# ArroyoSystems/arroyo

Measured on NVIDIA H100. Metric: rows/sec sliding-window SUM (1M keys), higher is better.
Workload: dtype int64

## Files before the change

arroyo_b200/csrc/ingest_two_pass.cuh:

```cuda
#pragma once

struct alignas(16) Rec {
  long long key;
  long long val;
};

constexpr int TP_NP = 2;
#ifndef AB_P1_THREADS
#define AB_P1_THREADS 512
#endif
#ifndef AB_P1_RPT
#define AB_P1_RPT 8
#endif
constexpr int P1_THREADS = AB_P1_THREADS;
constexpr int P1_RPT = AB_P1_RPT;
constexpr int P1_TILE = P1_THREADS * P1_RPT;
constexpr int P1_NWARP = P1_THREADS / 32;
constexpr int P1_NR = 1024;
constexpr int P1_BLOCKS_PER_SM = P1_TILE <= 4096 ? 2 : 1;
constexpr int P2_NW = 16;
constexpr int P2_NST = 3;
constexpr int P2_CH = 64;
constexpr int P2_BLOCKS_PER_SM = 2;
constexpr uint32_t NO_REGION = 0xFFFFu;

struct TwoPassParams {
  unsigned long long fast_q[TP_NP];
  unsigned long long* fast_ptr[TP_NP];
  uint32_t fast_slot[TP_NP];
  Rec* part;
  unsigned int* cursor;
  unsigned int* cursor_next;
  uint32_t cap;
  uint32_t slices;
  uint32_t tail_first;
  uint32_t tail_slices;
};

constexpr size_t P1_SMEM = (size_t)P1_TILE * 16 + (size_t)P1_NR * 12;
constexpr size_t P2_SMEM = (size_t)4096 * 11 + (size_t)BD_CAPB * 12 + (size_t)P2_NW * P2_NST * P2_CH * 16 +
                           (size_t)(P2_NW * P2_NST + 1) * 8;

template <int NV>
__device__ __noinline__ void direct_rec(const IngestParams& p, unsigned long long* pane, uint32_t slot, uint64_t q,
                                        long long key, long long val) {
  if (NV > 0 && p.guard_vals && big_one(val)) {
    atomicAdd(&p.counters->big_vals, 1ull);
// ... 132 lines not shown
#pragma unroll
    for (int o = 1; o < 32; o <<= 1) {
      const uint32_t y = __shfl_up_sync(0xffffffffu, incl, o);
      if (lane >= o) incl += y;
    }
    if (lane == 31) s_wsum[w] = incl;
    __syncthreads();
    uint32_t wbase = 0, n_on = 0;
#pragma unroll
    for (int ww = 0; ww < P1_NWARP; ++ww) {
      const uint32_t x = s_wsum[ww];
      if (ww < w) wbase += x;
      n_on += x;
    }
    const uint32_t ex0 = wbase + incl - tsum;
    uint32_t g[BPT];
    {
      uint32_t ex = ex0;
      const uint32_t rbase = (uint32_t)max(psel, 0) * NB;
#pragma unroll
      for (int x = 0; x < BPT; ++x) {
        const uint32_t b = BPT * tid + x;
        toff[b] = ex;
        g[x] = 0;
        if (c[x]) g[x] = atomicAdd(tp.cursor + rbase + b, c[x]);
        ex += c[x];
      }
    }
    __syncthreads();

// ... 12 lines not shown
        gdelta[BPT * tid + x] = g[x] - ex;
        ex += c[x];
      }
    }
    __syncthreads();
    if (n_on) {
      Rec* out = tp.part + (size_t)max(psel, 0) * NB * tp.cap;
      for (uint32_t i = tid; i < n_on; i += P1_THREADS) {
        const Rec rec = reorder[i];
        const uint32_t r = bd_bucket(bd_hash(rec.key), NB);
        const uint32_t dst = gdelta[r] + i;
        if (dst < tp.cap) {
          out[(size_t)r * tp.cap + dst] = rec;
        } else {
          atomicAdd(&p.counters->part_overflow, 1ull);
          direct_rec<NV>(p, fpane, fslot, tq, rec.key, rec.val);
        }
      }
    }
  }

  unsigned long long wl = late;
#pragma unroll
  for (int o = 16; o > 0; o >>= 1) {
    wl += __shfl_xor_sync(0xffffffffu, wl, o);
    maxq = max(maxq, __shfl_xor_sync(0xffffffffu, maxq, o));
  }
  if (lane == 0) {
    if (wl) atomicAdd(&s_late, wl);
    if (maxq) atomicMax(&s_maxq, (unsigned long long)maxq);
// ... 94 lines not shown
  uint32_t sl = (g + P2_HG) & (P2_HS - 1);
#pragma unroll 1
  for (int probe = 0; full && probe < P2_HS; ++probe) {
    const unsigned long long e = hk[sl];
    if (e == (unsigned long long)key && htag[sl] != 0) return hidx[sl];
    if (e == (unsigned long long)EMPTY_KEY) break;
    sl = (sl + 1) & (P2_HS - 1);
  }
  const uint32_t id = bd_insert(p.dict, b, key, bd_slot0(key));
  if (id >= ID_OVERFLOW) return ID_OVERFLOW;
  const uint32_t idx = id - bd_id(b, 0);
  p2_insert(hk, htag, hidx, key, idx);
  return idx;
}

__device__ __noinline__ void agg_defer(const IngestParams& p, long long key, long long ts, long long val, int why) {
  if (why == 0) atomicAdd(&p.counters->big_vals, 1ull);
  else atomicAdd(&p.counters->dict_full, 1u);
  defer_row(p, key, ts, val, 0, 0, 0);
}

constexpr unsigned P2_FLUSH_ITERS = 31;

template <int NV>
__global__ void __launch_bounds__(P2_NW * 32, P2_BLOCKS_PER_SM) agg_kernel(const __grid_constant__ IngestParams p,
                                                                           const __grid_constant__ TwoPassParams tp) {
  extern __shared__ __align__(128) unsigned char smem_raw[];
  unsigned long long* hk = reinterpret_cast<unsigned long long*>(smem_raw);
  unsigned char* htag = reinterpret_cast<unsigned char*>(hk + P2_HS);
  unsigned short* hidx = reinterpret_cast<unsigned short*>(htag + P2_HS);
  uint32_t* scw = reinterpret_cast<uint32_t*>(hidx + P2_HS);
  uint32_t* slo = scw + BD_CAPB;
  uint32_t* shi = slo + BD_CAPB;
  Rec* ring = reinterpret_cast<Rec*>(shi + BD_CAPB);
  unsigned long long* bars = reinterpret_cast<unsigned long long*>(ring + (size_t)P2_NW * P2_NST * P2_CH);
  __shared__ unsigned long long s_rows;
  const int tid = threadIdx.x, lane = tid & 31, w = tid >> 5;
  const uint32_t NB = p.dict.n_buckets;
  Rec* myring = ring + (size_t)w * P2_NST * P2_CH;
  const uint32_t bar0 = smem_u32(bars + (size_t)w * P2_NST);
  const uint32_t a_hk = smem_u32(hk), a_tag = smem_u32(htag), a_idx = smem_u32(hidx), a_cw = smem_u32(scw),
                 a_lo = smem_u32(slo), a_hi = smem_u32(shi), a_ring = smem_u32(myring);
  if (lane == 0)
    for (int s = 0; s < P2_NST; ++s) mbar_init(bar0 + 8 * s, 1);
  asm volatile("fence.mbarrier_init.release.cluster;" ::: "memory");
  for (int i = tid; i < 3 * BD_CAPB; i += P2_NW * 32) scw[i] = 0;
  if (tid == 0) s_rows = 0;
  __syncthreads();
  uint32_t phase = 0;
  const bool guard = NV > 0 && p.guard_vals != 0;

  const uint32_t head_work = tp.tail_first * tp.slices;
  const uint32_t n_work = head_work + (NB - tp.tail_first) * tp.tail_slices;
  for (uint32_t work = blockIdx.x; work < n_work; work += gridDim.x) {
    const bool tail = work >= head_work;
    const uint32_t n_slices = tail ? tp.tail_slices : tp.slices;
    const uint32_t b = tail ? tp.tail_first + (work - head_work) / n_slices : work / n_slices;
    const uint32_t slice = tail ? (work - head_work) % n_slices : work % n_slices;
    unsigned n_reg[TP_NP];
    unsigned n_any = 0;
#pragma unroll
    for (int f = 0; f < TP_NP; ++f) {
      n_reg[f] = tp.fast_ptr[f] ? min(tp.cursor[f * NB + b], tp.cap) : 0u;
      n_any |= n_reg[f];
      if (tid == 0) tp.cursor_next[f * NB + b] = 0;
    }
    if (n_any == 0) continue;

    const Rec* rows = nullptr;
    unsigned n = 0, my_chunks = 0;
    auto select = [&](int f) {
      const unsigned chunks_all = (n_reg[f] + P2_CH - 1) / P2_CH;
      const unsigned c_lo = (unsigned)((unsigned long long)chunks_all * slice / n_slices);
      const unsigned c_hi = (unsigned)((unsigned long long)chunks_all * (slice + 1) / n_slices);
      const unsigned r_lo = c_lo * P2_CH, r_hi = min(c_hi * P2_CH, n_reg[f]);
      rows = tp.part + (size_t)(f * NB + b) * tp.cap + r_lo;
      n = r_hi > r_lo ? r_hi - r_lo : 0u;
      const unsigned n_chunks = (n + P2_CH - 1) / P2_CH;
      my_chunks = n_chunks > (unsigned)w ? (n_chunks - w + P2_NW - 1) / P2_NW : 0;
    };
// ... 21 lines not shown
      }
    }
    __syncthreads();

#pragma unroll 1
    for (int f = 0; f < TP_NP; ++f) {
      if (f > 0) {
        select(f);
        for (unsigned ci = 0; ci < (unsigned)P2_NST && ci < my_chunks; ++ci) issue(ci, (int)ci);
      }
      if (n == 0) continue;
      unsigned long long* pane = tp.fast_ptr[f];
      const long long pane_ts = (long long)(tp.fast_q[f] * (uint64_t)p.slide);
      unsigned long long* prow = pane + bd_id(b, 0);
      unsigned long long* psum = pane + p.id_cap + bd_id(b, 0);
      unsigned int flushed = 0;
      auto flush = [&]() {
        for (unsigned i = tid; i < (unsigned)BD_CAPB; i += P2_NW * 32) {
          const uint32_t cw = scw[i];
          if (cw) {
            const uint32_t c = cw & 0xFFFFu;
            const uint32_t dh = (uint32_t)((int32_t)(cw - c) >> 16);
            const unsigned long long sum = ((unsigned long long)(shi[i] + dh) << 32) + (unsigned long long)slo[i];
            scw[i] = 0;
            slo[i] = 0;
            shi[i] = 0;
            flushed += c;
            if (n_slices == 1) {
              prow[i] += c;
              if (NV > 0) psum[i] += sum;
            } else {
              red_add_u64(prow + i, c);
              if (NV > 0) red_add_u64(psum + i, sum);
            }
          }
        }
      };
      const unsigned iters = ((n + P2_CH - 1) / P2_CH + P2_NW - 1) / P2_NW;
#pragma unroll 1
      for (unsigned ci = 0; ci < iters; ++ci) {
        if (ci && ci % P2_FLUSH_ITERS == 0) {
          __syncthreads();
          flush();
          __syncthreads();
        }
        if (ci >= my_chunks) continue;
        const int s = (int)(ci % P2_NST);
        mbar_wait(bar0 + 8 * s, (phase >> s) & 1u);
        phase ^= 1u << s;
// ... 15 lines not shown
            while (m) {
              const uint32_t bit = (uint32_t)__ffs(m) - 1u;
              m &= m - 1;
              const uint32_t j = (bit >> 3) + (bit & 4u);
              if ((uint32_t)((tg >> (8 * j)) & 0xFFull) != (tag4 & 0xFFu)) continue;
              const uint32_t sl = g + j;
              if (lds64(a_hk + sl * 8) == (unsigned long long)key) {
                idx = lds16(a_idx + sl * 2);
                break;
              }
            }
            if (idx == ID_UNSET) idx = agg_slow_lookup(p, hk, htag, hidx, b, key, g);
            const uint32_t vl = rr.z, vh = rr.w;
            const bool narrow = NV == 0 || (uint32_t)((int32_t)vl >> 31) == vh;
            if (idx >= (uint32_t)BD_CAPB) {
              agg_defer(p, key, pane_ts, (long long)(((unsigned long long)vh << 32) | vl), 1);
            } else if (NV > 0 && guard && !narrow) {
              agg_defer(p, key, pane_ts, (long long)(((unsigned long long)vh << 32) | vl), 0);
            } else if (NV == 0) {
              reds_add(a_cw + idx * 4, 1u);
            } else {
              const uint32_t old = atoms_add(a_lo + idx * 4, vl);
              uint32_t d = (old + vl) < vl ? 1u : 0u;
              if (narrow) d -= vl >> 31;
              else reds_add(a_hi + idx * 4, vh);
              reds_add(a_cw + idx * 4, 1u + (d << 16));
            }
          }
        }
        __syncwarp();
        if (ci + P2_NST < my_chunks) issue(ci + P2_NST, s);
      }
      __syncthreads();
      flush();
      flushed = __reduce_add_sync(0xffffffffu, flushed);
      if (lane == 0 && flushed) atomicAdd(&s_rows, (unsigned long long)flushed);
      __syncthreads();
      if (tid == 0) {
        if (s_rows) atomicAdd(p.slot_rows + tp.fast_slot[f], s_rows);
        s_rows = 0;
      }
    }
    __syncthreads();
  }
}
```

arroyo_b200/csrc/window_agg.cu:

```cuda
#include <algorithm>
#include <climits>
#include <deque>
#include <map>
#include <memory>
#include <set>

#include "agg_plan.h"
#include "bdict.cuh"
#include "op.h"
#include "planner.h"

namespace ab {
namespace {

constexpr int MAX_SEGS = 512;
constexpr int MAX_RING = 4096;
constexpr int RING_INLINE = 64;
constexpr int MAX_MERGE = 4096;
constexpr long long FREE_BIN = LLONG_MIN;

constexpr int THREADS = 256;
constexpr int PAIRS = 2;
constexpr int TILE = THREADS * PAIRS * 2;

// ... 682 lines not shown
  int slot = -1;
  bool in_tier = false;
  uint64_t rows = 0;
  bool exported = false;
  bool delta_exported = false;
};

struct LaunchRec {
  cudaEvent_t done = nullptr;
  cudaEvent_t t0 = nullptr, t1 = nullptr;
  Counters* h_counters = nullptr;
  unsigned long long* h_slot_rows = nullptr;
  uint64_t rows = 0;
  bool in_flight = false;
  int chunk = -1;
};

constexpr size_t RELEASE_GROUP = 16;
struct PendingRelease {
  cudaEvent_t ev;
  std::vector<ArrowArray> arrs;
};

class WindowAggOp final : public OpBase {
 public:
  explicit WindowAggOp(const ArroyoB200OpConfig& c);
  ~WindowAggOp() override;

  void on_start(ArrowArray* state, ArrowSchema* schemas, int64_t n, int64_t watermark, int64_t table_min) override;
  void process_batch(uint32_t, uint32_t, ArrowArray* batch, const ArrowSchema* schema) override;
// ... 28 lines not shown
  static constexpr size_t BOOK_SLOT_OFF = (sizeof(Counters) + 15) / 16 * 16;
  Counters* d_counters() const { return reinterpret_cast<Counters*>(book_.p); }
  unsigned long long* d_slot_rows() const { return reinterpret_cast<unsigned long long*>((char*)book_.p + BOOK_SLOT_OFF); }
  std::vector<unsigned long long> slot_rows_seen_;
  uint32_t n_keys_host_ = 1;
  uint32_t total_keys_host_ = 0;
  uint32_t dict_full_seen_ = 0;
  DevBuf part_, part_cursor_;
  uint32_t part_cap_ = 0;
  int part_flip_ = 0;
  bool two_pass_attr_set_ = false;
  bool two_pass_enabled_ = true;
  uint64_t part_overflow_seen_ = 0;
  mutable int two_pass_pause_ = 0;
  bool two_pass_eligible(uint64_t rows) const;
  void launch_two_pass(IngestParams& p, uint64_t rows, long long tiles_direct);
  BDict dict_view() const;
  cudaStream_t out_stream_ = nullptr;
  cudaEvent_t emit_done_ = nullptr, out_done_ = nullptr;
  bool async_out_ = false, out_inflight_ = false;
  void wait_outputs();
  static constexpr size_t COPY_GROUP = 48;
  std::vector<void*> copy_dst_, copy_src_;
  std::vector<size_t> copy_size_;
  bool batch_copy_ok_ = true;
  void queue_copy(void* dst, const void* src, size_t bytes);
  void flush_copies();
  std::vector<ArrowArray> open_release_;
  std::vector<cudaEvent_t> ev_pool_;
  void seal_release();

// ... 72 lines not shown
  void preallocate();
  void grow_ids();
  void apply_l2_policy();
  void promote_avg();
  void relayout_blocks(int old_n_acc, const std::vector<std::pair<int, int>>& f64_from);
  unsigned long long* acquire_block();
  void release_block(unsigned long long* blk);
  void init_block(unsigned long long* blk, uint64_t n_ids);
  void ensure_pane(int64_t bin);
  void drop_pane(int64_t bin);
  void upload_ring();
  void add_segment(const long long* key, const long long* ts, const long long* const* vals, int64_t n);
  void launch_pending();
  void launch_segments(const std::vector<Segment>& segs, int chunk);
  void absorb(int li);
  void sync_all();
  void drain_deferred();
  void poll_releases(bool wait);
  void rotate_chunk();
  void touch(int64_t bin);
  OutSet* out_set(size_t i, uint64_t cap);
  int64_t run_emit(const std::vector<const unsigned long long*>& blocks, int n_add, bool use_running, bool partial,
                   int64_t wstart, int64_t wend, int64_t ts, OutSet* os);
  void emit_window(int64_t a, int64_t b, size_t out_index, BatchesPriv* out_host,
                   std::vector<ArroyoB200DeviceBatch>* out_dev);
  void export_window(OutSet* os, int64_t n, BatchesPriv* out_host);
  void export_partial(OutSet* os, int64_t n, BatchesPriv* out);
  void collect_emit_times();
  void lookahead();
};

// ... 36 lines not shown

  book_.alloc(BOOK_SLOT_OFF + MAX_RING * sizeof(unsigned long long));
  AB_CUDA(cudaMemsetAsync(book_.p, 0, book_.bytes, stream_));
  slot_rows_seen_.assign(MAX_RING, 0);
  Counters init{};
  init.max_q = 0;
  init.n_keys = 0;
  AB_CUDA(cudaMemcpyAsync(book_.p, &init, sizeof init, cudaMemcpyHostToDevice, stream_));
  last_counters_ = init;

  uint64_t want = c.expected_keys ? c.expected_keys : (1ull << 16);
  alloc_dictionary(plan_.keyed ? bd_buckets_for(want) : 1);
  {
    const char* e = getenv("ARROYO_B200_NO_TWO_PASS");
    two_pass_enabled_ = !(e && atoi(e) != 0) && !(c.flags & ARROYO_B200_FLAG_NO_TWO_PASS);
  }

  h_pane_bins_.assign(MAX_RING, FREE_BIN);
  h_pane_ptrs_.assign(MAX_RING, nullptr);
  d_pane_bins_.alloc(MAX_RING * sizeof(long long));
  d_pane_ptrs_.alloc(MAX_RING * sizeof(void*));
  if (sliding_) {
    uint64_t need = (uint64_t)(width_ / slide_) + 8;
    while (ring_ < need && ring_ < MAX_RING) ring_ <<= 1;
  }

  const int n_used = 2 + plan_.n_vals;
  for (int i = 0; i < NCHUNK; ++i) {
    AB_CUDA(cudaEventCreateWithFlags(&chunk_free_[i], cudaEventDisableTiming));
    if (i == 0) {
// ... 36 lines not shown
    auto* blk = pane_storage_.back().as<unsigned long long>();
    init_block(blk, id_cap_);
    free_panes_.emplace_back(blk, 0);
  }
  for (int c = 0; c < 2 + plan_.n_vals; ++c) defer_[0][c].alloc(defer_cap_ * 8);
  out_set(0, id_cap_);
  out_set(1, id_cap_);
}

WindowAggOp::~WindowAggOp() {
  cudaSetDevice(device_);
  if (counts_done_) cudaEventDestroy(counts_done_);
  if (copy_stream_) cudaStreamSynchronize(copy_stream_);
  if (out_stream_) cudaStreamSynchronize(out_stream_);
  cudaStreamSynchronize(stream_);
  for (auto& r : releases_) {
    for (auto& a : r.arrs)
      if (a.release) a.release(&a);
    cudaEventDestroy(r.ev);
  }
  for (auto& a : zero_copy_inputs_)
    if (a.release) a.release(&a);
  for (auto& a : open_release_)
    if (a.release) a.release(&a);
  for (auto e : ev_pool_) cudaEventDestroy(e);
  for (int i = 0; i < NCHUNK; ++i)
    if (chunk_free_[i]) cudaEventDestroy(chunk_free_[i]);
  if (copy_stream_) {
    cudaStreamSynchronize(copy_stream_);
    cudaStreamDestroy(copy_stream_);
// ... 98 lines not shown

__global__ void permute_block_kernel(const unsigned long long* __restrict__ old_blk, unsigned long long* __restrict__ new_blk,
                                     const uint32_t* __restrict__ map, uint32_t old_ids, uint64_t old_cap, uint64_t new_cap,
                                     int n_acc) {
  uint32_t i = blockIdx.x * blockDim.x + threadIdx.x;
  const uint32_t stride = gridDim.x * blockDim.x;
  for (; i < old_ids; i += stride) {
    const uint32_t m = map[i];
    if (m == ID_UNSET || m >= ID_OVERFLOW) continue;
    for (int a = 0; a < n_acc; ++a) new_blk[(uint64_t)a * new_cap + m] = old_blk[(uint64_t)a * old_cap + i];
  }
}

void WindowAggOp::grow_ids() {
  AB_REQUIRE(plan_.keyed, ARROYO_B200_RUNTIME, "grow_ids on an unkeyed aggregate");
  const uint64_t old_cap = id_cap_;
  const uint32_t old_ids = n_keys_host_;
  BDict old_d = dict_view();
  DevBuf old_slots = std::move(slots_), old_nkeys = std::move(bucket_nkeys_), old_keys = std::move(id_keys_);
  old_d.slots = old_slots.as<BSlot>();
  old_d.nkeys = old_nkeys.as<unsigned int>();
  old_d.id_keys = old_keys.as<long long>();
  const unsigned int zero = 0;
  AB_CUDA(cudaMemcpyAsync((char*)book_.p + offsetof(Counters, n_keys), &zero, sizeof zero, cudaMemcpyHostToDevice, stream_));
  alloc_dictionary(n_buckets_ * 2);
  const uint64_t new_cap = id_cap_;
  DevBuf map((size_t)old_cap * sizeof(uint32_t));
  {
    const int grid = (int)std::min<uint64_t>((old_ids + 255) / 256, (uint64_t)num_sms_ * 8);
    bd_rehash_kernel<<<std::max(grid, 1), 256, 0, stream_>>>(old_d, dict_view(), old_ids, map.as<uint32_t>());
// ... 65 lines not shown
  }
  for (auto& kv : zombies_) {
    kv.second.dev = migrate(kv.second.dev);
    kv.second.frozen = migrate(kv.second.frozen);
  }
  running_ = migrate(running_);
  AB_CUDA(cudaStreamSynchronize(stream_));
  free_panes_.clear();
  pane_storage_ = std::move(new_storage);
  ring_dirty_ = true;
}

void WindowAggOp::promote_avg() {
  if (!avg_exact_) return;
  AB_REQUIRE(in_flight_.empty(), ARROYO_B200_RUNTIME, "promote with launches in flight");
  const int old_n_acc = plan_.n_acc;
  std::set<int> avg_srcs;
  for (int g = 0; g < plan_.n_aggs; ++g)
    if (plan_.agg_kind[g] == ARROYO_B200_AGG_AVG_I64) avg_srcs.insert(plan_.agg_acc[g]);
  AB_REQUIRE(old_n_acc + (int)avg_srcs.size() <= MAX_ACC, ARROYO_B200_RUNTIME, "too many accumulators after AVG promotion");
  std::vector<std::pair<int, int>> f64_from;
  for (int g = 0; g < plan_.n_aggs; ++g) {
    if (plan_.agg_kind[g] != ARROYO_B200_AGG_AVG_I64) continue;
    const int src = plan_.agg_acc[g];
    int found = -1;
    for (auto& pr : f64_from)
      if (pr.second == src) found = pr.first;
    if (found < 0) {
      found = plan_.n_acc;
      plan_.acc_kind[plan_.n_acc] = ACC_SUM_F64;
// ... 14 lines not shown
    zombies_.clear();
    release_block(running_);
    running_ = nullptr;
  }
  relayout_blocks(old_n_acc, f64_from);
}

void WindowAggOp::ensure_pane(int64_t bin) {
  auto it = panes_.find(bin);
  if (it != panes_.end() && it->second.slot >= 0) return;
  const uint64_t q = (uint64_t)bin / (uint64_t)slide_;
  uint32_t slot;
  while (true) {
    slot = (uint32_t)q & (ring_ - 1);
    if (h_pane_bins_[slot] == FREE_BIN) break;
    if (ring_ == MAX_RING) {
      auto old = panes_.find(h_pane_bins_[slot]);
      AB_REQUIRE(old != panes_.end(), ARROYO_B200_RUNTIME, "ring slot of an unknown pane");
      old->second.slot = -1;
      h_pane_bins_[slot] = FREE_BIN;
      h_pane_ptrs_[slot] = nullptr;
      ring_dirty_ = true;
      break;
    }
    ring_ *= 2;
    std::fill(h_pane_bins_.begin(), h_pane_bins_.end(), FREE_BIN);
    std::fill(h_pane_ptrs_.begin(), h_pane_ptrs_.end(), nullptr);
    for (auto& kv : panes_) {
      if (kv.second.slot < 0) continue;
      uint32_t s = (uint32_t)((uint64_t)kv.first / (uint64_t)slide_) & (ring_ - 1);
// ... 244 lines not shown
  if (!two_pass_enabled_ || !plan_.keyed || rows_slot_ >= 0 || plan_.n_vals > 1 || plan_.n_acc > 2) return false;
  if (plan_.n_acc == 2 && plan_.acc_kind[1] != ACC_SUM_I64) return false;
  if (n_buckets_ > (uint64_t)P1_NR) return false;
  if (max_bin_seen_ == LLONG_MIN) return false;
  if (two_pass_pause_ > 0) {
    --two_pass_pause_;
    return false;
  }
  static const uint64_t min_rows = [] {
    const char* e = getenv("ARROYO_B200_TWO_PASS_MIN_ROWS");
    return e ? strtoull(e, nullptr, 10) : (1ull << 19);
  }();
  return rows >= min_rows || (cfg.flags & ARROYO_B200_FLAG_TWO_PASS_ALWAYS);
}

void WindowAggOp::launch_two_pass(IngestParams& p, uint64_t rows, long long tiles) {
  TwoPassParams tp{};
  int nf = 0;
  for (int k = 0; k < 3 && nf < TP_NP; ++k) {
    const int64_t b = max_bin_seen_ + (int64_t)(k == 2 ? -1 : k) * slide_;
    auto it = panes_.find(b);
    if (b < late_bin_ || it == panes_.end() || it->second.slot < 0) continue;
    tp.fast_q[nf] = (unsigned long long)b / (unsigned long long)slide_;
    tp.fast_ptr[nf] = it->second.dev;
    tp.fast_slot[nf] = (uint32_t)it->second.slot;
    ++nf;
  }
  for (int f = nf; f < TP_NP; ++f) {
    tp.fast_q[f] = ~0ull;
    tp.fast_ptr[f] = nullptr;
    tp.fast_slot[f] = 0;
  }
  const uint32_t n_regions = (uint32_t)(TP_NP * n_buckets_);
  const uint64_t mean = (uint64_t)launch_rows_ / n_buckets_ + 1;
  const uint32_t cap = (uint32_t)std::min<uint64_t>(((mean + mean / 4 + 2048 + 63) / 64) * 64, 1u << 30);
  if (part_cap_ != cap || !part_.p) {
    AB_CUDA(cudaStreamSynchronize(stream_));
    part_.alloc((size_t)n_regions * cap * sizeof(Rec));
    part_cursor_.alloc((size_t)2 * n_regions * sizeof(unsigned int));
    AB_CUDA(cudaMemsetAsync(part_cursor_.p, 0, (size_t)2 * n_regions * sizeof(unsigned int), stream_));
    part_cap_ = cap;
  }
  tp.part = part_.as<Rec>();
  tp.cursor = part_cursor_.as<unsigned int>() + (size_t)part_flip_ * n_regions;
  tp.cursor_next = part_cursor_.as<unsigned int>() + (size_t)(part_flip_ ^ 1) * n_regions;
  part_flip_ ^= 1;
  tp.cap = cap;
  const uint32_t want_blocks = (uint32_t)num_sms_ * 2;
  tp.slices = (uint32_t)std::max<uint64_t>(1, std::min<uint64_t>((want_blocks + n_buckets_ - 1) / n_buckets_,
                                                                 std::max<uint64_t>(1, rows / n_buckets_ / 4096)));
  if (!two_pass_attr_set_) {
    AB_CUDA(cudaFuncSetAttribute(part_kernel<0, 0>, cudaFuncAttributeMaxDynamicSharedMemorySize, (int)P1_SMEM));
    AB_CUDA(cudaFuncSetAttribute(part_kernel<1, sig_of(ACC_SUM_I64)>, cudaFuncAttributeMaxDynamicSharedMemorySize, (int)P1_SMEM));
    AB_CUDA(cudaFuncSetAttribute(agg_kernel<0>, cudaFuncAttributeMaxDynamicSharedMemorySize, (int)P2_SMEM));
    AB_CUDA(cudaFuncSetAttribute(agg_kernel<1>, cudaFuncAttributeMaxDynamicSharedMemorySize, (int)P2_SMEM));
    two_pass_attr_set_ = true;
  }
  const int grid1 = (int)std::max<long long>(1, std::min<long long>(tiles, (long long)num_sms_ * P1_BLOCKS_PER_SM));
  const uint32_t max_blocks = (uint32_t)num_sms_ * P2_BLOCKS_PER_SM;
  tp.tail_first = (uint32_t)n_buckets_;
  tp.tail_slices = 1;
  if (tp.slices == 1 && n_buckets_ > max_blocks && rows / n_buckets_ >= 2048) {
    const uint32_t rest = (uint32_t)(n_buckets_ % max_blocks);
    if (rest && max_blocks / rest >= 2) {
      tp.tail_first = (uint32_t)n_buckets_ - rest;
      tp.tail_slices = std::min<uint32_t>(max_blocks / rest, 4);
    }
  }
  const uint32_t n_work = tp.tail_first * tp.slices + ((uint32_t)n_buckets_ - tp.tail_first) * tp.tail_slices;
  const int grid2 = (int)std::max<uint32_t>(1, std::min<uint32_t>(n_work, max_blocks));
  if (plan_.n_vals == 0) {
    part_kernel<0, 0><<<grid1, P1_THREADS, P1_SMEM, stream_>>>(p, tp);
    AB_CUDA(cudaGetLastError());
    agg_kernel<0><<<grid2, P2_NW * 32, P2_SMEM, stream_>>>(p, tp);
  } else {
    part_kernel<1, sig_of(ACC_SUM_I64)><<<grid1, P1_THREADS, P1_SMEM, stream_>>>(p, tp);
    AB_CUDA(cudaGetLastError());
    agg_kernel<1><<<grid2, P2_NW * 32, P2_SMEM, stream_>>>(p, tp);
  }
  ++st_.kernel_launches;
}

void WindowAggOp::launch_segments(const std::vector<Segment>& segs_in, int chunk) {
  while (in_flight_.size() >= 2) absorb(in_flight_.front());
  if (!draining_ && have_counters_ && last_counters_.deferred > 0) {
    while (!in_flight_.empty()) absorb(in_flight_.front());
    drain_deferred();
  }
  const int li = next_launch_;
  next_launch_ = (next_launch_ + 1) % NLAUNCH;
  LaunchRec& L = launches_[li];
  AB_REQUIRE(!L.in_flight, ARROYO_B200_RUNTIME, "launch record still in flight");
  Segment* hs = h_segs_[li].as<Segment>();
  long long tiles = 0;
  uint64_t rows = 0;
  for (size_t i = 0; i < segs_in.size(); ++i) {
    hs[i] = segs_in[i];
    hs[i].tile_start = tiles;
    uintptr_t al = (uintptr_t)hs[i].ts;
// ... 35 lines not shown
    }
  for (int a = 0; a < plan_.n_acc; ++a) {
    p.acc_kind[a] = plan_.acc_kind[a];
    p.acc_val[a] = plan_.acc_val[a];
  }
  p.counters = d_counters();
  p.slot_rows = d_slot_rows();
  p.d_key = defer_[defer_cur_][0].as<long long>();
  p.d_ts = defer_[defer_cur_][1].as<long long>();
  for (int v = 0; v < plan_.n_vals; ++v) p.d_val[v] = defer_[defer_cur_][2 + v].as<long long>();
  p.defer_cap = defer_cap_;

  int grid = (int)std::min<long long>(tiles, (long long)num_sms_ * 8);
  if (grid < 1) grid = 1;
  if (profile_) AB_CUDA(cudaEventRecord(L.t0, stream_));
  const bool two_pass = two_pass_eligible(rows);
  if (two_pass) {
    long long t2 = 0;
    for (size_t i = 0; i < segs_in.size(); ++i) {
      hs[i].tile_start = t2;
      t2 += (hs[i].n + P1_TILE - 1) / P1_TILE;
    }
    AB_CUDA(cudaMemcpyAsync(d_segs_[li].p, hs, segs_in.size() * sizeof(Segment), cudaMemcpyHostToDevice, stream_));
    p.n_tiles = t2;
    launch_two_pass(p, rows, t2);
  }
  int sig = GENERIC_SIG;
  if (plan_.n_vals <= 1 && plan_.n_acc <= 4) {
    int k[3] = {0, 0, 0};
    for (int a = 1; a < plan_.n_acc; ++a) k[a - 1] = plan_.acc_kind[a];
    sig = sig_of(k[0], k[1], k[2]);
  }
#define AB_LAUNCH(NV, SIG) ingest_kernel<NV, SIG><<<grid, THREADS, 0, stream_>>>(p)
  if (two_pass) {
  } else if (plan_.n_vals == 0) AB_LAUNCH(0, 0);
  else if (plan_.n_vals == 1 && sig == sig_of(ACC_SUM_I64)) AB_LAUNCH(1, sig_of(ACC_SUM_I64));
  else if (plan_.n_vals == 1 && sig == sig_of(ACC_SUM_F64)) AB_LAUNCH(1, sig_of(ACC_SUM_F64));
  else if (plan_.n_vals == 1 && sig == sig_of(ACC_SUM_I64, ACC_SUM_F64)) AB_LAUNCH(1, sig_of(ACC_SUM_I64, ACC_SUM_F64));
  else if (plan_.n_vals == 1 && sig == sig_of(ACC_MIN_I64, ACC_MAX_I64)) AB_LAUNCH(1, sig_of(ACC_MIN_I64, ACC_MAX_I64));
  else if (plan_.n_vals == 1) AB_LAUNCH(1, GENERIC_SIG);
  else if (plan_.n_vals == 2) AB_LAUNCH(2, GENERIC_SIG);
  else if (plan_.n_vals == 3) AB_LAUNCH(3, GENERIC_SIG);
  else AB_LAUNCH(4, GENERIC_SIG);
#undef AB_LAUNCH
  AB_CUDA(cudaGetLastError());
  if (profile_) AB_CUDA(cudaEventRecord(L.t1, stream_));
  ++st_.kernel_launches;
  ++st_.ingest_launches;
  AB_CUDA(cudaMemcpyAsync(L.h_counters, book_.p, BOOK_SLOT_OFF + ring_ * sizeof(unsigned long long), cudaMemcpyDeviceToHost,
                          stream_));
  AB_CUDA(cudaEventRecord(L.done, stream_));
  if (chunk >= 0) AB_CUDA(cudaEventRecord(chunk_free_[chunk], stream_));
  L.rows = rows;
  L.in_flight = true;
  L.chunk = chunk;
  in_flight_.push_back(li);
}

void WindowAggOp::launch_pending() {
  seal_release();
  if (segs_.empty()) return;
  std::vector<Segment> segs;
  segs.swap(segs_);
// ... 20 lines not shown
}

void WindowAggOp::touch(int64_t bin) {
  if (sliding_) sliding_planner_->touch(bin);
  else tumbling_->touch(bin);
}

void WindowAggOp::absorb(int li) {
  LaunchRec& L = launches_[li];
  AB_REQUIRE(L.in_flight, ARROYO_B200_RUNTIME, "absorb of an idle launch");
  AB_CUDA(cudaEventSynchronize(L.done));
  L.in_flight = false;
  AB_REQUIRE(!in_flight_.empty() && in_flight_.front() == li, ARROYO_B200_RUNTIME, "launch order violated");
  in_flight_.pop_front();
  if (profile_) {
    float ms = 0;
    AB_CUDA(cudaEventElapsedTime(&ms, L.t0, L.t1));
    st_.ingest_ms += ms;
    st_.ingest_rows_timed += L.rows;
  }
  const Counters& c = *L.h_counters;
  last_counters_ = c;
  have_counters_ = true;
  total_keys_host_ = c.n_keys;
  if (c.part_overflow != part_overflow_seen_) {
    if (c.part_overflow - part_overflow_seen_ > L.rows / 64) two_pass_pause_ = 64;
    part_overflow_seen_ = c.part_overflow;
  }
  if (c.max_q) max_bin_seen_ = std::max<int64_t>(max_bin_seen_, (int64_t)(c.max_q * (uint64_t)slide_));
  for (uint32_t s = 0; s < ring_; ++s) {
    const unsigned long long fresh = L.h_slot_rows[s] - slot_rows_seen_[s];
    slot_rows_seen_[s] = L.h_slot_rows[s];
    if (fresh) {
      AB_REQUIRE(h_pane_bins_[s] != FREE_BIN, ARROYO_B200_RUNTIME, "touched a free ring slot");
      Pane& tp = panes_.at(h_pane_bins_[s]);
      tp.rows += fresh;
      if (tp.rows >= (1ull << 31)) need_promote_ = true;
      touch(h_pane_bins_[s]);
    }
  }
  if (c.lost) throw Error(ARROYO_B200_RUNTIME, "deferred-row buffer overflowed; rows were lost");
  if (c.neg_ts)
    throw Error(ARROYO_B200_PANIC, "batch holds a negative _timestamp (before the Unix epoch): the reference panics on it");
  lookahead();
}

void WindowAggOp::lookahead() {
  if (max_bin_seen_ == LLONG_MIN) return;
  for (int k = 0; k <= 2; ++k) {
    int64_t b = max_bin_seen_ + (int64_t)k * slide_;
    if (b >= late_bin_ && !panes_.count(b)) {
      uint32_t slot = (uint32_t)((uint64_t)b / (uint64_t)slide_) & (ring_ - 1);
      if (h_pane_bins_[slot] == FREE_BIN) ensure_pane(b);
    }
  }
}

void WindowAggOp::sync_all() {
  while (!in_flight_.empty()) absorb(in_flight_.front());
  if (need_promote_ && avg_exact_) promote_avg();
  drain_deferred();
}

void WindowAggOp::drain_deferred() {
  struct Guard {
    bool& f;
    explicit Guard(bool& x) : f(x) { f = true; }
    ~Guard() { f = false; }
  } guard(draining_);
  uint64_t prev = UINT64_MAX;
  for (int stalls = 0; stalls < 64;) {
    if (!have_counters_ || last_counters_.deferred == 0) return;
    AB_REQUIRE(in_flight_.empty(), ARROYO_B200_RUNTIME, "drain with launches in flight");
    const uint64_t n = last_counters_.deferred;
    stalls = n < prev ? 0 : stalls + 1;
    prev = n;
    AB_REQUIRE(n <= defer_cap_, ARROYO_B200_RUNTIME, "deferred overflow");
    st_.rows_deferred += n;
    std::vector<long long> ts(n);
    AB_CUDA(cudaMemcpyAsync(ts.data(), defer_[defer_cur_][1].p, n * 8, cudaMemcpyDeviceToHost, stream_));
    AB_CUDA(cudaStreamSynchronize(stream_));
    std::set<int64_t> bins;
    for (uint64_t i = 0; i < n; ++i) {
      int64_t b = (int64_t)((uint64_t)ts[i] / (uint64_t)slide_ * (uint64_t)slide_);
// ... 6 lines not shown
      dict_full_seen_ = last_counters_.dict_full;
      grow_ids();
      last_counters_.n_keys = total_keys_host_;
    }
    const int full = defer_cur_;
    defer_cur_ ^= 1;
    unsigned long long zero = 0;
    AB_CUDA(cudaMemcpyAsync((char*)book_.p + offsetof(Counters, deferred), &zero, sizeof zero,
                            cudaMemcpyHostToDevice, stream_));
    Segment s{};
    s.key = defer_[full][0].as<long long>();
    s.ts = defer_[full][1].as<long long>();
    for (int v = 0; v < plan_.n_vals; ++v) s.val[v] = defer_[full][2 + v].as<long long>();
    s.n = (long long)n;
    launch_segments({s}, -1);
    while (!in_flight_.empty()) absorb(in_flight_.front());
  }
  throw Error(ARROYO_B200_RUNTIME, "deferred rows did not converge");
}

void WindowAggOp::flush() {
  set_device();
  resolve_deferred();
  launch_pending();
  sync_all();
  poll_releases(true);
}

void WindowAggOp::submit() {
  set_device();
  launch_pending();
}

void WindowAggOp::wait_outputs() {
  if (!out_inflight_) return;
  AB_CUDA(cudaEventSynchronize(out_done_));
  out_inflight_ = false;
}

void WindowAggOp::begin_watermark(int64_t wm) {
// ... 215 lines not shown
  for (size_t ci : fix_f64) {
    long long* raw = (long long*)cols[ci].data;
    double* d = (double*)cols[ci].data;
    for (int64_t i = 0; i < n; ++i) d[i] = (double)raw[i];
  }
  out->arrays.emplace_back();
  out->schemas.emplace_back();
  export_batch(cols, n, &out->arrays.back(), &out->schemas.back());
}

void WindowAggOp::emit_window(int64_t a, int64_t b, size_t out_index, BatchesPriv* out_host,
                              std::vector<ArroyoB200DeviceBatch>* out_dev) {
  std::vector<int64_t> members;
  for (auto it = panes_.lower_bound(a); it != panes_.end() && it->first < b; ++it)
    if (it->second.in_tier) members.push_back(it->first);
  if (avg_exact_ && guard_vals_) {
    uint64_t window_rows = 0;
    for (int64_t m : members) window_rows += panes_.at(m).rows;
    if (window_rows >= (1ull << 32)) promote_avg();
  }
  std::vector<const unsigned long long*> blocks;
  int n_add = 0;
  bool use_running = false;
  if (running_mode_) {
    if (!running_) {
      running_ = acquire_block();
    }
    std::set<int64_t> target(members.begin(), members.end());
    std::vector<const unsigned long long*> add, sub;
    for (int64_t m : target)
// ... 53 lines not shown
      cols.insert(cols.begin() + wi, (uint64_t)os->wstart.p);
    }
    cols.push_back((uint64_t)os->ts.p);
    for (uint64_t v : cols) d.cols[c++] = v;
    d.n_cols = c;
    out_dev->push_back(d);
  }
}

void WindowAggOp::handle_watermark(int64_t wm, BatchesPriv* out_host, std::vector<ArroyoB200DeviceBatch>* out_dev) {
  set_device();
  if (!defer_counts_) resolve_deferred();
  wait_outputs();
  launch_pending();
  sync_all();
  poll_releases(false);
  std::vector<PlanStep> steps;
  if (sliding_) sliding_planner_->watermark(wm, steps);
  else tumbling_->watermark(wm, steps);
  size_t out_index = 0;
  for (const PlanStep& s : steps) {
    switch (s.kind) {
      case PlanStep::JOIN: {
        auto it = panes_.find(s.a);
        AB_REQUIRE(it != panes_.end(), ARROYO_B200_RUNTIME, "closing a pane that is not resident");
        it->second.in_tier = true;
        break;
      }
      case PlanStep::EMIT: {
        if (!sliding_) {
// ... 104 lines not shown
  if (!profile_ || emit_events_used_ == 0) return;
  AB_CUDA(cudaEventSynchronize(emit_events_[emit_events_used_ - 1].second));
  for (size_t i = 0; i < emit_events_used_; ++i) {
    float ms = 0;
    AB_CUDA(cudaEventElapsedTime(&ms, emit_events_[i].first, emit_events_[i].second));
    st_.emit_ms += ms;
  }
  emit_events_used_ = 0;
}

void WindowAggOp::handle_checkpoint(int64_t wm, BatchesPriv* out) {
  set_device();
  resolve_deferred();
  wait_outputs();
  launch_pending();
  sync_all();
  std::vector<PlanStep> steps;
  if (sliding_) sliding_planner_->checkpoint(wm != INT64_MIN, wm, steps);
  else tumbling_->checkpoint(steps);
  for (const PlanStep& s : steps) {
    if (s.kind != PlanStep::CHECKPOINT_PANE) continue;
    auto it = panes_.find(s.a);
    AB_REQUIRE(it != panes_.end(), ARROYO_B200_RUNTIME, "checkpointing a pane that is not resident");
    Pane& p = it->second;
    OutSet* os = out_set(0, std::max<uint64_t>(n_keys_host_, 1));
    int64_t n = run_emit({p.dev}, 1, false, true, 0, 0, s.a, os);
    if (n > 0) export_partial(os, n, out);
    p.delta_exported = true;
    if (!p.frozen) p.frozen = acquire_block();
    FoldParams fp{};
    fp.active = p.dev;
// ... 11 lines not shown
    Pane& p = kv.second;
    if (!p.in_tier || p.exported) continue;
    std::vector<const unsigned long long*> blocks{p.dev};
    if (p.frozen && !p.delta_exported) blocks.push_back(p.frozen);
    OutSet* os = out_set(0, std::max<uint64_t>(n_keys_host_, 1));
    int64_t n = run_emit(blocks, (int)blocks.size(), false, true, 0, 0, kv.first, os);
    if (n > 0) export_partial(os, n, out);
    p.exported = true;
  }
  AB_CUDA(cudaStreamSynchronize(stream_));
  collect_emit_times();
}

void WindowAggOp::on_start(ArrowArray* state, ArrowSchema* schemas, int64_t n, int64_t watermark, int64_t table_min) {
  set_device();
  const bool has_wm = watermark != INT64_MIN;
  if (has_wm) late_bin_ = std::max<int64_t>(late_bin_, bin_start(watermark, slide_));
  if (sliding_) sliding_planner_->restore_begin(has_wm, watermark);
  int n_state_cols = 0;
  for (int g = 0; g < plan_.n_aggs; ++g) n_state_cols += plan_.agg_kind[g] == ARROYO_B200_AGG_AVG_I64 ? 2 : 1;
  const int expect_cols = (plan_.keyed ? 1 : 0) + n_state_cols + 1;
  std::vector<DevBuf> keep;
  for (int64_t bi = 0; bi < n; ++bi) {
    int64_t rows = 0;
    std::vector<InColumn> cols = import_batch(&state[bi], &schemas[bi], &rows);
    AB_REQUIRE((int)cols.size() == expect_cols, ARROYO_B200_INVALID_ARGUMENT,
               "state batch does not match the partial schema");
    if (rows == 0) continue;
    if (plan_.keyed) key_format_ = cols[0].format;
    const int64_t ts = (int64_t)cols.back().data[0];
// ... 77 lines not shown
    AB_CUDA(cudaMemcpyAsync(&c, book_.p, sizeof c, cudaMemcpyDeviceToHost, stream_));
    AB_CUDA(cudaStreamSynchronize(stream_));
    AB_REQUIRE(c.lost == 0, ARROYO_B200_RUNTIME, "dictionary overflow during restore");
    total_keys_host_ = c.n_keys;
    last_counters_ = c;
    max_bin_seen_ = std::max<int64_t>(max_bin_seen_, bin);
    if (state[bi].release) state[bi].release(&state[bi]);
  }
  if (sliding_) sliding_planner_->restore_end(table_min != INT64_MIN, table_min);
  AB_CUDA(cudaStreamSynchronize(stream_));
}

void WindowAggOp::stats(ArroyoB200Stats* out) {
  set_device();
  resolve_deferred();
  st_.n_keys = plan_.keyed ? total_keys_host_ : 0;
  st_.rows_late = last_counters_.late_rows;
  *out = st_;
}

}

OpBase* make_window_agg_op(const ArroyoB200OpConfig& cfg) { return new WindowAggOp(cfg); }

}
```

Before: 22.63 billion.

## Overlap two-pass aggregation kernel with next ingest on a second stream

Moves the aggregation pass of the two-pass ingest onto a separate stream and double-buffers the partition buffers and cursors. The next batch's partition kernel can then run while the previous aggregation is still in flight. Row accounting per slot moves from the agg kernel to the partition kernel, which drops the shared-memory row reduction and the non-atomic single-slice flush path. The cursor reset becomes a memset after each agg launch. A settle() step joins the streams before dictionary growth, emits, checkpoints and ring-slot reuse. This adds host-side synchronisation logic and doubles the partition buffer memory.

Result: faster. 24.78 billion (median of 6 runs) (+9.5%).

```diff
diff --git a/arroyo_b200/csrc/ingest_two_pass.cuh b/arroyo_b200/csrc/ingest_two_pass.cuh
--- a/arroyo_b200/csrc/ingest_two_pass.cuh
+++ b/arroyo_b200/csrc/ingest_two_pass.cuh
@@ -30,7 +30,6 @@
   uint32_t fast_slot[TP_NP];
   Rec* part;
   unsigned int* cursor;
-  unsigned int* cursor_next;
   uint32_t cap;
   uint32_t slices;
   uint32_t tail_first;
@@ -193,6 +192,7 @@
       n_on += x;
     }
     const uint32_t ex0 = wbase + incl - tsum;
+    if (tid == 0 && n_on) atomicAdd(p.slot_rows + fslot, (unsigned long long)n_on);
     uint32_t g[BPT];
     {
       uint32_t ex = ex0;
@@ -235,6 +235,7 @@
           out[(size_t)r * tp.cap + dst] = rec;
         } else {
           atomicAdd(&p.counters->part_overflow, 1ull);
+          atomicAdd(p.slot_rows + fslot, ~0ull);
           direct_rec<NV>(p, fpane, fslot, tq, rec.key, rec.val);
         }
       }
@@ -359,9 +360,10 @@
   return idx;
 }
 
-__device__ __noinline__ void agg_defer(const IngestParams& p, long long key, long long ts, long long val, int why) {
+__device__ __noinline__ void agg_defer(const IngestParams& p, uint32_t slot, long long key, long long ts, long long val, int why) {
   if (why == 0) atomicAdd(&p.counters->big_vals, 1ull);
   else atomicAdd(&p.counters->dict_full, 1u);
+  atomicAdd(p.slot_rows + slot, ~0ull);
   defer_row(p, key, ts, val, 0, 0, 0);
 }
 
@@ -379,7 +381,6 @@
   uint32_t* shi = slo + BD_CAPB;
   Rec* ring = reinterpret_cast<Rec*>(shi + BD_CAPB);
   unsigned long long* bars = reinterpret_cast<unsigned long long*>(ring + (size_t)P2_NW * P2_NST * P2_CH);
-  __shared__ unsigned long long s_rows;
   const int tid = threadIdx.x, lane = tid & 31, w = tid >> 5;
   const uint32_t NB = p.dict.n_buckets;
   Rec* myring = ring + (size_t)w * P2_NST * P2_CH;
@@ -390,7 +391,6 @@
     for (int s = 0; s < P2_NST; ++s) mbar_init(bar0 + 8 * s, 1);
   asm volatile("fence.mbarrier_init.release.cluster;" ::: "memory");
   for (int i = tid; i < 3 * BD_CAPB; i += P2_NW * 32) scw[i] = 0;
-  if (tid == 0) s_rows = 0;
   __syncthreads();
   uint32_t phase = 0;
   const bool guard = NV > 0 && p.guard_vals != 0;
@@ -408,7 +408,6 @@
     for (int f = 0; f < TP_NP; ++f) {
       n_reg[f] = tp.fast_ptr[f] ? min(tp.cursor[f * NB + b], tp.cap) : 0u;
       n_any |= n_reg[f];
-      if (tid == 0) tp.cursor_next[f * NB + b] = 0;
     }
     if (n_any == 0) continue;
 
@@ -460,7 +459,6 @@
       const long long pane_ts = (long long)(tp.fast_q[f] * (uint64_t)p.slide);
       unsigned long long* prow = pane + bd_id(b, 0);
       unsigned long long* psum = pane + p.id_cap + bd_id(b, 0);
-      unsigned int flushed = 0;
       auto flush = [&]() {
         for (unsigned i = tid; i < (unsigned)BD_CAPB; i += P2_NW * 32) {
           const uint32_t cw = scw[i];
@@ -471,14 +469,8 @@
             scw[i] = 0;
             slo[i] = 0;
             shi[i] = 0;
-            flushed += c;
-            if (n_slices == 1) {
-              prow[i] += c;
-              if (NV > 0) psum[i] += sum;
-            } else {
-              red_add_u64(prow + i, c);
-              if (NV > 0) red_add_u64(psum + i, sum);
-            }
+            red_add_u64(prow + i, c);
+            if (NV > 0) red_add_u64(psum + i, sum);
           }
         }
       };
@@ -524,9 +516,9 @@
             const uint32_t vl = rr.z, vh = rr.w;
             const bool narrow = NV == 0 || (uint32_t)((int32_t)vl >> 31) == vh;
             if (idx >= (uint32_t)BD_CAPB) {
-              agg_defer(p, key, pane_ts, (long long)(((unsigned long long)vh << 32) | vl), 1);
+              agg_defer(p, tp.fast_slot[f], key, pane_ts, (long long)(((unsigned long long)vh << 32) | vl), 1);
             } else if (NV > 0 && guard && !narrow) {
-              agg_defer(p, key, pane_ts, (long long)(((unsigned long long)vh << 32) | vl), 0);
+              agg_defer(p, tp.fast_slot[f], key, pane_ts, (long long)(((unsigned long long)vh << 32) | vl), 0);
             } else if (NV == 0) {
               reds_add(a_cw + idx * 4, 1u);
             } else {
@@ -543,14 +535,8 @@
       }
       __syncthreads();
       flush();
-      flushed = __reduce_add_sync(0xffffffffu, flushed);
-      if (lane == 0 && flushed) atomicAdd(&s_rows, (unsigned long long)flushed);
       __syncthreads();
-      if (tid == 0) {
-        if (s_rows) atomicAdd(p.slot_rows + tp.fast_slot[f], s_rows);
-        s_rows = 0;
-      }
-    }
-    __syncthreads();
-  }
-}
+    }
+    __syncthreads();
+  }
+}
diff --git a/arroyo_b200/csrc/window_agg.cu b/arroyo_b200/csrc/window_agg.cu
--- a/arroyo_b200/csrc/window_agg.cu
+++ b/arroyo_b200/csrc/window_agg.cu
@@ -720,6 +720,9 @@
   uint64_t rows = 0;
   bool in_flight = false;
   int chunk = -1;
+  bool agg_overlapped = false;
+  int n_agg_bins = 0;
+  int64_t agg_bins[TP_NP] = {};
 };
 
 constexpr size_t RELEASE_GROUP = 16;
@@ -778,7 +781,19 @@
   uint64_t part_overflow_seen_ = 0;
   mutable int two_pass_pause_ = 0;
   bool two_pass_eligible(uint64_t rows) const;
-  void launch_two_pass(IngestParams& p, uint64_t rows, long long tiles_direct);
+  void launch_two_pass(IngestParams& p, uint64_t rows, long long tiles_direct, LaunchRec& L);
+  bool ingest_overlap_ = true;
+  cudaStream_t agg_stream_ = nullptr;
+  cudaEvent_t part_done_ = nullptr;
+  cudaEvent_t agg_done_[2] = {nullptr, nullptr};
+  bool agg_used_[2] = {false, false};
+  int agg_open_set_ = -1;
+  std::vector<int64_t> open_bins_;
+  PinnedBuf h_settle_;
+  int timing_pending_ = -1;
+  void settle();
+  void fold_counters(const Counters& c, const unsigned long long* slot_rows, uint64_t rows);
+  void collect_ingest_time(int li);
   BDict dict_view() const;
   cudaStream_t out_stream_ = nullptr;
   cudaEvent_t emit_done_ = nullptr, out_done_ = nullptr;
@@ -881,7 +896,7 @@
   void launch_pending();
   void launch_segments(const std::vector<Segment>& segs, int chunk);
   void absorb(int li);
-  void sync_all();
+  void sync_all(bool settle_agg = false);
   void drain_deferred();
   void poll_releases(bool wait);
   void rotate_chunk();
@@ -948,6 +963,16 @@
   {
     const char* e = getenv("ARROYO_B200_NO_TWO_PASS");
     two_pass_enabled_ = !(e && atoi(e) != 0) && !(c.flags & ARROYO_B200_FLAG_NO_TWO_PASS);
+    const char* o = getenv("ARROYO_B200_INGEST_OVERLAP");
+    ingest_overlap_ = two_pass_enabled_ && !(o && atoi(o) == 0);
+  }
+  if (ingest_overlap_) {
+    int prio = 0;
+    AB_CUDA(cudaStreamGetPriority(stream_, &prio));
+    AB_CUDA(cudaStreamCreateWithPriority(&agg_stream_, cudaStreamNonBlocking, prio));
+    AB_CUDA(cudaEventCreateWithFlags(&part_done_, cudaEventDisableTiming));
+    for (auto& e : agg_done_) AB_CUDA(cudaEventCreateWithFlags(&e, cudaEventDisableTiming));
+    h_settle_.alloc(BOOK_SLOT_OFF + MAX_RING * sizeof(unsigned long long));
   }
 
   h_pane_bins_.assign(MAX_RING, FREE_BIN);
@@ -1014,6 +1039,12 @@
   if (copy_stream_) cudaStreamSynchronize(copy_stream_);
   if (out_stream_) cudaStreamSynchronize(out_stream_);
   cudaStreamSynchronize(stream_);
+  if (agg_stream_) {
+    cudaStreamSynchronize(agg_stream_);
+    cudaStreamDestroy(agg_stream_);
+    cudaEventDestroy(part_done_);
+    for (auto e : agg_done_) cudaEventDestroy(e);
+  }
   for (auto& r : releases_) {
     for (auto& a : r.arrs)
       if (a.release) a.release(&a);
@@ -1142,6 +1173,7 @@
 
 void WindowAggOp::grow_ids() {
   AB_REQUIRE(plan_.keyed, ARROYO_B200_RUNTIME, "grow_ids on an unkeyed aggregate");
+  settle();
   const uint64_t old_cap = id_cap_;
   const uint32_t old_ids = n_keys_host_;
   BDict old_d = dict_view();
@@ -1237,6 +1269,7 @@
 void WindowAggOp::promote_avg() {
   if (!avg_exact_) return;
   AB_REQUIRE(in_flight_.empty(), ARROYO_B200_RUNTIME, "promote with launches in flight");
+  settle();
   const int old_n_acc = plan_.n_acc;
   std::set<int> avg_srcs;
   for (int g = 0; g < plan_.n_aggs; ++g)
@@ -1281,6 +1314,7 @@
   while (true) {
     slot = (uint32_t)q & (ring_ - 1);
     if (h_pane_bins_[slot] == FREE_BIN) break;
+    settle();
     if (ring_ == MAX_RING) {
       auto old = panes_.find(h_pane_bins_[slot]);
       AB_REQUIRE(old != panes_.end(), ARROYO_B200_RUNTIME, "ring slot of an unknown pane");
@@ -1555,7 +1589,7 @@
   return rows >= min_rows || (cfg.flags & ARROYO_B200_FLAG_TWO_PASS_ALWAYS);
 }
 
-void WindowAggOp::launch_two_pass(IngestParams& p, uint64_t rows, long long tiles) {
+void WindowAggOp::launch_two_pass(IngestParams& p, uint64_t rows, long long tiles, LaunchRec& L) {
   TwoPassParams tp{};
   int nf = 0;
   for (int k = 0; k < 3 && nf < TP_NP; ++k) {
@@ -1575,17 +1609,20 @@
   const uint32_t n_regions = (uint32_t)(TP_NP * n_buckets_);
   const uint64_t mean = (uint64_t)launch_rows_ / n_buckets_ + 1;
   const uint32_t cap = (uint32_t)std::min<uint64_t>(((mean + mean / 4 + 2048 + 63) / 64) * 64, 1u << 30);
+  const int n_sets = ingest_overlap_ ? 2 : 1;
   if (part_cap_ != cap || !part_.p) {
+    settle();
     AB_CUDA(cudaStreamSynchronize(stream_));
-    part_.alloc((size_t)n_regions * cap * sizeof(Rec));
-    part_cursor_.alloc((size_t)2 * n_regions * sizeof(unsigned int));
-    AB_CUDA(cudaMemsetAsync(part_cursor_.p, 0, (size_t)2 * n_regions * sizeof(unsigned int), stream_));
+    part_.alloc((size_t)n_sets * n_regions * cap * sizeof(Rec));
+    part_cursor_.alloc((size_t)n_sets * n_regions * sizeof(unsigned int));
+    AB_CUDA(cudaMemsetAsync(part_cursor_.p, 0, (size_t)n_sets * n_regions * sizeof(unsigned int), stream_));
     part_cap_ = cap;
-  }
-  tp.part = part_.as<Rec>();
-  tp.cursor = part_cursor_.as<unsigned int>() + (size_t)part_flip_ * n_regions;
-  tp.cursor_next = part_cursor_.as<unsigned int>() + (size_t)(part_flip_ ^ 1) * n_regions;
+    agg_used_[0] = agg_used_[1] = false;
+  }
+  const int set = part_flip_ % n_sets;
   part_flip_ ^= 1;
+  tp.part = part_.as<Rec>() + (size_t)set * n_regions * cap;
+  tp.cursor = part_cursor_.as<unsigned int>() + (size_t)set * n_regions;
   tp.cap = cap;
   const uint32_t want_blocks = (uint32_t)num_sms_ * 2;
   tp.slices = (uint32_t)std::max<uint64_t>(1, std::min<uint64_t>((want_blocks + n_buckets_ - 1) / n_buckets_,
@@ -1610,20 +1647,34 @@
   }
   const uint32_t n_work = tp.tail_first * tp.slices + ((uint32_t)n_buckets_ - tp.tail_first) * tp.tail_slices;
   const int grid2 = (int)std::max<uint32_t>(1, std::min<uint32_t>(n_work, max_blocks));
-  if (plan_.n_vals == 0) {
-    part_kernel<0, 0><<<grid1, P1_THREADS, P1_SMEM, stream_>>>(p, tp);
-    AB_CUDA(cudaGetLastError());
-    agg_kernel<0><<<grid2, P2_NW * 32, P2_SMEM, stream_>>>(p, tp);
-  } else {
-    part_kernel<1, sig_of(ACC_SUM_I64)><<<grid1, P1_THREADS, P1_SMEM, stream_>>>(p, tp);
-    AB_CUDA(cudaGetLastError());
-    agg_kernel<1><<<grid2, P2_NW * 32, P2_SMEM, stream_>>>(p, tp);
+  if (ingest_overlap_ && agg_used_[set]) AB_CUDA(cudaStreamWaitEvent(stream_, agg_done_[set], 0));
+  if (plan_.n_vals == 0) part_kernel<0, 0><<<grid1, P1_THREADS, P1_SMEM, stream_>>>(p, tp);
+  else part_kernel<1, sig_of(ACC_SUM_I64)><<<grid1, P1_THREADS, P1_SMEM, stream_>>>(p, tp);
+  AB_CUDA(cudaGetLastError());
+  cudaStream_t s2 = stream_;
+  if (ingest_overlap_) {
+    AB_CUDA(cudaEventRecord(part_done_, stream_));
+    AB_CUDA(cudaStreamWaitEvent(agg_stream_, part_done_, 0));
+    s2 = agg_stream_;
+  }
+  if (plan_.n_vals == 0) agg_kernel<0><<<grid2, P2_NW * 32, P2_SMEM, s2>>>(p, tp);
+  else agg_kernel<1><<<grid2, P2_NW * 32, P2_SMEM, s2>>>(p, tp);
+  AB_CUDA(cudaGetLastError());
+  AB_CUDA(cudaMemsetAsync(tp.cursor, 0, (size_t)n_regions * sizeof(unsigned int), s2));
+  if (ingest_overlap_) {
+    if (profile_) AB_CUDA(cudaEventRecord(L.t1, agg_stream_));
+    AB_CUDA(cudaEventRecord(agg_done_[set], agg_stream_));
+    agg_used_[set] = true;
+    agg_open_set_ = set;
+    L.agg_overlapped = true;
+    L.n_agg_bins = nf;
+    for (int f = 0; f < nf; ++f) L.agg_bins[f] = (int64_t)(tp.fast_q[f] * (unsigned long long)slide_);
   }
   ++st_.kernel_launches;
 }
 
 void WindowAggOp::launch_segments(const std::vector<Segment>& segs_in, int chunk) {
-  while (in_flight_.size() >= 2) absorb(in_flight_.front());
+  while (in_flight_.size() >= (ingest_overlap_ ? 1u : 2u)) absorb(in_flight_.front());
   if (!draining_ && have_counters_ && last_counters_.deferred > 0) {
     while (!in_flight_.empty()) absorb(in_flight_.front());
     drain_deferred();
@@ -1689,6 +1740,9 @@
   int grid = (int)std::min<long long>(tiles, (long long)num_sms_ * 8);
   if (grid < 1) grid = 1;
   if (profile_) AB_CUDA(cudaEventRecord(L.t0, stream_));
+  const int open_before = agg_open_set_;
+  L.agg_overlapped = false;
+  L.n_agg_bins = 0;
   const bool two_pass = two_pass_eligible(rows);
   if (two_pass) {
     long long t2 = 0;
@@ -1698,7 +1752,7 @@
     }
     AB_CUDA(cudaMemcpyAsync(d_segs_[li].p, hs, segs_in.size() * sizeof(Segment), cudaMemcpyHostToDevice, stream_));
     p.n_tiles = t2;
-    launch_two_pass(p, rows, t2);
+    launch_two_pass(p, rows, t2, L);
   }
   int sig = GENERIC_SIG;
   if (plan_.n_vals <= 1 && plan_.n_acc <= 4) {
@@ -1719,9 +1773,13 @@
   else AB_LAUNCH(4, GENERIC_SIG);
 #undef AB_LAUNCH
   AB_CUDA(cudaGetLastError());
-  if (profile_) AB_CUDA(cudaEventRecord(L.t1, stream_));
+  if (profile_ && !L.agg_overlapped) AB_CUDA(cudaEventRecord(L.t1, stream_));
   ++st_.kernel_launches;
   ++st_.ingest_launches;
+  if (open_before >= 0) {
+    AB_CUDA(cudaStreamWaitEvent(stream_, agg_done_[open_before], 0));
+    if (agg_open_set_ == open_before) agg_open_set_ = -1;
+  }
   AB_CUDA(cudaMemcpyAsync(L.h_counters, book_.p, BOOK_SLOT_OFF + ring_ * sizeof(unsigned long long), cudaMemcpyDeviceToHost,
                           stream_));
   AB_CUDA(cudaEventRecord(L.done, stream_));
@@ -1772,35 +1830,64 @@
   AB_REQUIRE(!in_flight_.empty() && in_flight_.front() == li, ARROYO_B200_RUNTIME, "launch order violated");
   in_flight_.pop_front();
   if (profile_) {
-    float ms = 0;
-    AB_CUDA(cudaEventElapsedTime(&ms, L.t0, L.t1));
-    st_.ingest_ms += ms;
-    st_.ingest_rows_timed += L.rows;
-  }
-  const Counters& c = *L.h_counters;
+    if (timing_pending_ >= 0) collect_ingest_time(timing_pending_);
+    if (L.agg_overlapped) timing_pending_ = li;
+    else collect_ingest_time(li);
+  }
+  open_bins_.assign(L.agg_bins, L.agg_bins + L.n_agg_bins);
+  fold_counters(*L.h_counters, L.h_slot_rows, L.rows);
+  lookahead();
+}
+
+void WindowAggOp::collect_ingest_time(int li) {
+  const LaunchRec& L = launches_[li];
+  float ms = 0;
+  AB_CUDA(cudaEventSynchronize(L.t1));
+  AB_CUDA(cudaEventElapsedTime(&ms, L.t0, L.t1));
+  st_.ingest_ms += ms;
+  st_.ingest_rows_timed += L.rows;
+  if (timing_pending_ == li) timing_pending_ = -1;
+}
+
+void WindowAggOp::settle() {
+  while (!in_flight_.empty()) absorb(in_flight_.front());
+  if (agg_open_set_ < 0) return;
+  AB_CUDA(cudaStreamWaitEvent(stream_, agg_done_[agg_open_set_], 0));
+  agg_open_set_ = -1;
+  AB_CUDA(cudaMemcpyAsync(h_settle_.p, book_.p, BOOK_SLOT_OFF + ring_ * sizeof(unsigned long long), cudaMemcpyDeviceToHost,
+                          stream_));
+  AB_CUDA(cudaStreamSynchronize(stream_));
+  if (timing_pending_ >= 0) collect_ingest_time(timing_pending_);
+  open_bins_.clear();
+  fold_counters(*h_settle_.as<Counters>(),
+                reinterpret_cast<const unsigned long long*>((const char*)h_settle_.p + BOOK_SLOT_OFF), 0);
+}
+
+void WindowAggOp::fold_counters(const Counters& c, const unsigned long long* slot_rows, uint64_t rows) {
   last_counters_ = c;
   have_counters_ = true;
   total_keys_host_ = c.n_keys;
   if (c.part_overflow != part_overflow_seen_) {
-    if (c.part_overflow - part_overflow_seen_ > L.rows / 64) two_pass_pause_ = 64;
+    if (c.part_overflow - part_overflow_seen_ > rows / 64) two_pass_pause_ = 64;
     part_overflow_seen_ = c.part_overflow;
   }
   if (c.max_q) max_bin_seen_ = std::max<int64_t>(max_bin_seen_, (int64_t)(c.max_q * (uint64_t)slide_));
   for (uint32_t s = 0; s < ring_; ++s) {
-    const unsigned long long fresh = L.h_slot_rows[s] - slot_rows_seen_[s];
-    slot_rows_seen_[s] = L.h_slot_rows[s];
+    const long long fresh = (long long)(slot_rows[s] - slot_rows_seen_[s]);
+    slot_rows_seen_[s] = slot_rows[s];
     if (fresh) {
       AB_REQUIRE(h_pane_bins_[s] != FREE_BIN, ARROYO_B200_RUNTIME, "touched a free ring slot");
       Pane& tp = panes_.at(h_pane_bins_[s]);
-      tp.rows += fresh;
-      if (tp.rows >= (1ull << 31)) need_promote_ = true;
-      touch(h_pane_bins_[s]);
+      tp.rows += (uint64_t)fresh;
+      if (fresh > 0) {
+        if (tp.rows >= (1ull << 31)) need_promote_ = true;
+        touch(h_pane_bins_[s]);
+      }
     }
   }
   if (c.lost) throw Error(ARROYO_B200_RUNTIME, "deferred-row buffer overflowed; rows were lost");
   if (c.neg_ts)
     throw Error(ARROYO_B200_PANIC, "batch holds a negative _timestamp (before the Unix epoch): the reference panics on it");
-  lookahead();
 }
 
 void WindowAggOp::lookahead() {
@@ -1814,8 +1901,9 @@
   }
 }
 
-void WindowAggOp::sync_all() {
+void WindowAggOp::sync_all(bool settle_agg) {
   while (!in_flight_.empty()) absorb(in_flight_.front());
+  if (settle_agg) settle();
   if (need_promote_ && avg_exact_) promote_avg();
   drain_deferred();
 }
@@ -1826,6 +1914,8 @@
     explicit Guard(bool& x) : f(x) { f = true; }
     ~Guard() { f = false; }
   } guard(draining_);
+  if (!have_counters_ || last_counters_.deferred == 0) return;
+  settle();
   uint64_t prev = UINT64_MAX;
   for (int stalls = 0; stalls < 64;) {
     if (!have_counters_ || last_counters_.deferred == 0) return;
@@ -1862,7 +1952,7 @@
     for (int v = 0; v < plan_.n_vals; ++v) s.val[v] = defer_[full][2 + v].as<long long>();
     s.n = (long long)n;
     launch_segments({s}, -1);
-    while (!in_flight_.empty()) absorb(in_flight_.front());
+    settle();
   }
   throw Error(ARROYO_B200_RUNTIME, "deferred rows did not converge");
 }
@@ -1871,7 +1961,7 @@
   set_device();
   resolve_deferred();
   launch_pending();
-  sync_all();
+  sync_all(true);
   poll_releases(true);
 }
 
@@ -2117,6 +2207,8 @@
   std::vector<int64_t> members;
   for (auto it = panes_.lower_bound(a); it != panes_.end() && it->first < b; ++it)
     if (it->second.in_tier) members.push_back(it->first);
+  for (int64_t m : open_bins_)
+    AB_REQUIRE(m < a || m >= b, ARROYO_B200_RUNTIME, "emitting a pane whose aggregation pass may still be running");
   if (avg_exact_ && guard_vals_) {
     uint64_t window_rows = 0;
     for (int64_t m : members) window_rows += panes_.at(m).rows;
@@ -2200,6 +2292,11 @@
   wait_outputs();
   launch_pending();
   sync_all();
+  for (int64_t b : open_bins_)
+    if (b < bin_start(wm, slide_)) {
+      sync_all(true);
+      break;
+    }
   poll_releases(false);
   std::vector<PlanStep> steps;
   if (sliding_) sliding_planner_->watermark(wm, steps);
@@ -2334,7 +2431,7 @@
   resolve_deferred();
   wait_outputs();
   launch_pending();
-  sync_all();
+  sync_all(true);
   std::vector<PlanStep> steps;
   if (sliding_) sliding_planner_->checkpoint(wm != INT64_MIN, wm, steps);
   else tumbling_->checkpoint(steps);
@@ -2376,6 +2473,7 @@
 
 void WindowAggOp::on_start(ArrowArray* state, ArrowSchema* schemas, int64_t n, int64_t watermark, int64_t table_min) {
   set_device();
+  settle();
   const bool has_wm = watermark != INT64_MIN;
   if (has_wm) late_bin_ = std::max<int64_t>(late_bin_, bin_start(watermark, slide_));
   if (sliding_) sliding_planner_->restore_begin(has_wm, watermark);
@@ -2483,6 +2581,7 @@
 void WindowAggOp::stats(ArroyoB200Stats* out) {
   set_device();
   resolve_deferred();
+  if (agg_open_set_ >= 0) settle();
   st_.n_keys = plan_.keyed ? total_keys_host_ : 0;
   st_.rows_late = last_counters_.late_rows;
   *out = st_;
```
